# 0xPolygonZero/plonky

Measured on AMD Instinct MI355X. Metric: MSM Mpairs/sec + NTT Melems/sec, 2^20 Tweedledee, 1/2/4/8 GPU, higher is better.
Workload: dtype u32; 1 GPU; 2^20 TweedledeeBase forward NTT + 2^20-pair tweedledee MSM per GPU per step; log_n=20, curve=tweedledee

## Files before the change

### plonky_amd/csrc/msm_order.hip

```cpp
#include "msm_dev.cuh"
#include "glv.cuh"
#include <cstdlib>

namespace plk {


struct OrdRaw {
    uint4 lo, hi;
};
PLK_DI OrdRaw ord_load_scalar(const uint4* __restrict__ scalars, size_t i, bool live) {
    OrdRaw r;
    r.lo = r.hi = make_uint4(0u, 0u, 0u, 0u);
    if (live) {
        r.lo = scalars[i * 2];
        r.hi = scalars[i * 2 + 1];
    }
    return r;
}
template <class SP> PLK_DI void ord_park_loaded(const OrdRaw& r, uint32_t* s_lim, int tid, bool raw_signed) {
    static_assert(SP::NL == 8, "scalar fields are 256-bit");
    Fe<SP> s;
    s.v[0] = r.lo.x; s.v[1] = r.lo.y; s.v[2] = r.lo.z; s.v[3] = r.lo.w;
    s.v[4] = r.hi.x; s.v[5] = r.hi.y; s.v[6] = r.hi.z; s.v[7] = r.hi.w;
    if (!raw_signed) s = fe_to_canonical<SP>(s);
// ... 486 lines not shown
    __syncthreads();
    const uint32_t last_total = s_bins[nbins - 1];
    block_excl_scan4(s_bins, nbins, s_sum);
    for (int k = threadIdx.x; k < nbins; k += 256) bin_base[k] = s_bins[k];
    if (threadIdx.x == 0) {
        const uint32_t total = s_bins[nbins - 1] + last_total;
        bin_base[nbins] = total;
        uint32_t ch = lanes_cfg ? (total + lanes_cfg - 1) / lanes_cfg : chunk_cfg;
        if (ch < 8u) ch = 8u;
        if (ch > chunk_cfg) ch = chunk_cfg;
        dyn_chunk[0] = ch;
    }
    __syncthreads();
    for (int k = threadIdx.x; k < nbins; k += 256) s_bins[k] = s_tot[k] > hot ? (s_tot[k] + ORD_SEG - 1) / ORD_SEG : 0u;
    __syncthreads();
    const uint32_t last_segs = s_bins[nbins - 1];
    block_excl_scan4(s_bins, nbins, s_sum);
    for (int k = threadIdx.x; k < nbins; k += 256) seg_base[k] = s_bins[k];
    if (threadIdx.x == 0) seg_base[nbins] = s_bins[nbins - 1] + last_segs;
}

struct Ord2Seg {
    uint32_t bin, seg, plo, phi;
};
PLK_DI bool ord2_segment(const uint32_t* __restrict__ seg_base, const uint32_t* __restrict__ bin_base, int nbins, uint32_t blk, Ord2Seg& sg) {
    if (blk >= seg_base[nbins]) return false;
    uint32_t a = 0, b = (uint32_t)nbins;
    while (b - a > 1) {
        const uint32_t m = (a + b) >> 1;
        if (seg_base[m] <= blk) a = m; else b = m;
    }
    sg.bin = a;
    sg.seg = blk - seg_base[a];
    sg.plo = sg.seg * ORD_SEG;
    sg.phi = min(bin_base[a + 1] - bin_base[a], sg.plo + ORD_SEG);
    return true;
}
PLK_DI void ord2_prefix(const uint32_t* __restrict__ cnt1, uint32_t nt, uint32_t bin, uint32_t* s_run, uint32_t* s_pre, uint32_t* s_tmp) {
    const int tid = threadIdx.x, nthr = blockDim.x;
    const uint32_t per = (nt + nthr - 1) / nthr;
    const uint32_t lo = min(nt, (uint32_t)tid * per), hi = min(nt, lo + per);
    uint32_t sum = 0;
    for (uint32_t t = lo; t < hi; ++t) {
        const uint32_t w = cnt1[(size_t)bin * nt + t];
        s_run[t] = w;
        sum += w & 0xFFFFu;
    }
    uint32_t total = 0;
    uint32_t run = block_excl_prefix(sum, s_tmp, &total);
    for (uint32_t t = lo; t < hi; ++t) {
        s_pre[t] = run;
        run += s_run[t] & 0xFFFFu;
    }
    if (tid == 0) {
        s_pre[nt] = total;
        s_run[nt] = 0;
    }
    __syncthreads();
}
template <int THREADS = ORD_BIN_THREADS, int EPT = ORD_SEG_EPT>
PLK_DI void ord2_gather(const uint32_t* __restrict__ tmp, const uint32_t* s_run, const uint32_t* s_pre, uint32_t nt, uint32_t cap, uint32_t plo, uint32_t phi,
                        uint32_t (&rec)[EPT], uint32_t (&til)[EPT]) {
    uint32_t t[EPT];
#pragma unroll
    for (int k = 0; k < EPT; ++k) t[k] = 0;
    uint32_t top = 1;
    while (top * 2 <= nt) top *= 2;
    for (uint32_t step = top; step; step >>= 1) {
#pragma unroll
        for (int k = 0; k < EPT; ++k) {
            const uint32_t p = plo + threadIdx.x + (uint32_t)k * THREADS;
            const uint32_t cand = t[k] + step;
            if (cand < nt && s_pre[cand] <= p) t[k] = cand;
        }
    }
#pragma unroll
    for (int k = 0; k < EPT; ++k) {
        const uint32_t p = plo + threadIdx.x + (uint32_t)k * THREADS;
        til[k] = t[k];
        rec[k] = 0;
        if (p < phi) rec[k] = tmp[(size_t)t[k] * cap + (s_run[t[k]] >> 16) + (p - s_pre[t[k]])];
    }
}
__global__ void __launch_bounds__(ORD_BIN_THREADS) k_ord_bin_count2(const uint32_t* __restrict__ tmp, const uint32_t* __restrict__ cnt1, uint32_t nt, uint32_t cap,
                                                                    const uint32_t* __restrict__ bin_base, const uint32_t* __restrict__ seg_base, int fine_bits,
                                                                    int nbins, uint32_t* __restrict__ cnt2) {
    __shared__ uint32_t s_hist[1 << ORD_MAX_FINE];
    __shared__ uint32_t s_tmp[ORD_BIN_THREADS];
    extern __shared__ __attribute__((aligned(16))) uint32_t s_dyn[];
    uint32_t* s_run = s_dyn;
    uint32_t* s_pre = s_dyn + (nt + 1);
    const int tid = threadIdx.x;
    const int nf = 1 << fine_bits;
    const uint32_t fmask = (uint32_t)nf - 1u;
    for (uint32_t blk = blockIdx.x;; blk += gridDim.x) {
        Ord2Seg sg;
        if (!ord2_segment(seg_base, bin_base, nbins, blk, sg)) return;
        for (int k = tid; k < nf; k += ORD_BIN_THREADS) s_hist[k] = 0;
        ord2_prefix(cnt1, nt, sg.bin, s_run, s_pre, s_tmp);
        uint32_t rec[ORD_SEG_EPT], til[ORD_SEG_EPT];
        ord2_gather(tmp, s_run, s_pre, nt, cap, sg.plo, sg.phi, rec, til);
#pragma unroll
        for (int k = 0; k < ORD_SEG_EPT; ++k)
            if (sg.plo + tid + k * ORD_BIN_THREADS < sg.phi) atomicAdd(&s_hist[(rec[k] >> 1) & fmask], 1u);
        __syncthreads();
        for (int k = tid; k < nf; k += ORD_BIN_THREADS) cnt2[((size_t)blk << fine_bits) + k] = s_hist[k];
        __syncthreads();
    }
}
__global__ void __launch_bounds__(ORD_BIN_THREADS) k_ord_bin_scatter2(const uint32_t* __restrict__ tmp, const uint32_t* __restrict__ cnt1, uint32_t nt, uint32_t cap,
                                                                      const uint32_t* __restrict__ bin_base, const uint32_t* __restrict__ seg_base, int fine_bits,
                                                                      int nbins, uint32_t buckets, const uint32_t* __restrict__ cnt2, uint32_t* __restrict__ off,
                                                                      uint32_t* __restrict__ sorted, uint32_t entries_cap, uint32_t ent_stride, uint32_t ent_first) {
    __shared__ uint32_t s_tmp[ORD_BIN_THREADS];
    __shared__ uint32_t s_out[ORD_SEG];
    __shared__ uint16_t s_fine[ORD_SEG];
    extern __shared__ __attribute__((aligned(16))) uint32_t s_dyn[];
    uint32_t* s_glob = s_dyn;
    uint32_t* s_loc = s_dyn + ((size_t)1 << fine_bits);
    uint32_t* s_cur = s_dyn + ((size_t)2 << fine_bits);
    uint32_t* s_run = s_dyn + ((size_t)3 << fine_bits);
    uint32_t* s_pre = s_run + (nt + 1);
    const int tid = threadIdx.x;
    for (uint32_t blk = blockIdx.x;; blk += gridDim.x) {
    Ord2Seg sg;
    if (!ord2_segment(seg_base, bin_base, nbins, blk, sg)) return;
    const int nf = 1 << fine_bits;
    const uint32_t fmask = (uint32_t)nf - 1u;
    const uint32_t bin = sg.bin, seg = sg.seg;
    ord2_prefix(cnt1, nt, bin, s_run, s_pre, s_tmp);
    uint32_t rec[ORD_SEG_EPT], til[ORD_SEG_EPT];
    ord2_gather(tmp, s_run, s_pre, nt, cap, sg.plo, sg.phi, rec, til);
    const uint32_t s0 = seg_base[bin], s1 = seg_base[bin + 1];
    for (int k = tid; k < nf; k += ORD_BIN_THREADS) {
        uint32_t tot = 0, before = 0, own = 0;
        for (uint32_t sgi = s0; sgi < s1; ++sgi) {
            const uint32_t v = cnt2[((size_t)sgi << fine_bits) + k];
            if (sgi - s0 < seg) before += v;
            if (sgi - s0 == seg) own = v;
            tot += v;
        }
        s_glob[k] = tot;
        s_cur[k] = before;
        s_loc[k] = own;
    }
    __syncthreads();
    block_excl_scan4(s_glob, nf, s_tmp);
    block_excl_scan4(s_loc, nf, s_tmp);
    const uint32_t bb = bin_base[bin];
    for (int k = tid; k < nf; k += ORD_BIN_THREADS) {
        const uint32_t o = bb + s_glob[k];
        if (seg == 0) off[((size_t)bin << fine_bits) + k] = o;
        s_glob[k] = o + s_cur[k];
        s_cur[k] = s_loc[k];
    }
    __syncthreads();
#pragma unroll
    for (int k = 0; k < ORD_SEG_EPT; ++k) {
        if (sg.plo + tid + k * ORD_BIN_THREADS >= sg.phi) continue;
        const uint32_t r = rec[k];
        const uint32_t f = (r >> 1) & fmask;
        const uint32_t idx = atomicAdd(&s_cur[f], 1u);
        if (PLK_CHK(idx < ORD_SEG, CHK_SEG_STAGE)) {
            const uint32_t entry = ((r >> 12) & 15u) * ent_stride + ent_first + til[k] * (uint32_t)ORD2_TS + (r >> 16);
            s_out[idx] = (entry << 1) | (r & 1u);
            s_fine[idx] = (uint16_t)f;
        }
    }
    __syncthreads();
    const uint32_t count = sg.phi - sg.plo;
    for (uint32_t i = tid; i < count; i += ORD_BIN_THREADS) {
        const uint32_t f = s_fine[i];
        const uint32_t at = s_glob[f] + (i - s_loc[f]);
        if (PLK_CHK(at < entries_cap, CHK_SORTED_INDEX)) sorted[at] = s_out[i];
    }
    __syncthreads();
    }
}

constexpr int ORD2_SORT_THREADS = 1024;
constexpr int ORD2_SORT_UNROLL = 8;
template <class F>
PLK_DI void ord2_for_runs(const uint32_t* __restrict__ tmp, const uint32_t* s_run, uint32_t nt, uint32_t cap, F&& f) {
    const uint32_t hw = threadIdx.x >> 5, hl = threadIdx.x & 31u;
    constexpr uint32_t HW = ORD2_SORT_THREADS / 32;
    for (uint32_t t0 = hw; t0 < nt; t0 += HW * ORD2_SORT_UNROLL) {
        uint32_t w[ORD2_SORT_UNROLL], r[ORD2_SORT_UNROLL];
#pragma unroll
        for (int u = 0; u < ORD2_SORT_UNROLL; ++u) {
            const uint32_t t = t0 + (uint32_t)u * HW;
            w[u] = t < nt ? s_run[t] : 0u;
            r[u] = 0;
            if (hl < (w[u] & 0xFFFFu)) r[u] = tmp[(size_t)t * cap + (w[u] >> 16) + hl];
        }
#pragma unroll
        for (int u = 0; u < ORD2_SORT_UNROLL; ++u) {
            const uint32_t t = t0 + (uint32_t)u * HW, cnt = w[u] & 0xFFFFu;
            if (hl < cnt) f(r[u], t);
            for (uint32_t i = hl + 32u; i < cnt; i += 32u) f(tmp[(size_t)t * cap + (w[u] >> 16) + i], t);
        }
    }
}
template <bool CACHE>
__global__ void __launch_bounds__(ORD2_SORT_THREADS) k_ord_bin_sort(const uint32_t* __restrict__ tmp, const uint32_t* __restrict__ cnt1, uint32_t nt, uint32_t cap,
                                                                    const uint32_t* __restrict__ bin_base, int fine_bits, int nbins, uint32_t buckets,
                                                                    uint32_t* __restrict__ off, uint32_t* __restrict__ sorted, uint32_t entries_cap,
                                                                    uint32_t ent_stride, uint32_t ent_first) {
    __shared__ uint32_t s_tmp[ORD2_SORT_THREADS];
    extern __shared__ __attribute__((aligned(16))) uint32_t s_dyn[];
    const int nf = 1 << fine_bits;
    uint32_t* s_out = s_dyn;
    uint32_t* s_cur = s_dyn + ORD2_BIN_CAP;
    uint32_t* s_run = s_cur + nf;
    const int tid = threadIdx.x;
    const uint32_t bin = blockIdx.x;
    const uint32_t bb = bin_base[bin], total = bin_base[bin + 1] - bb;
    if (bin == 0 && tid == 0) off[buckets] = bin_base[nbins];
    if (total == 0) {
        for (int k = tid; k < nf; k += ORD2_SORT_THREADS) off[((size_t)bin << fine_bits) + k] = bb;
        return;
    }
    if (total > ORD2_BIN_CAP) return;
    const uint32_t fmask = (uint32_t)nf - 1u;
    for (int k = tid; k < nf; k += ORD2_SORT_THREADS) s_cur[k] = 0;
    for (uint32_t t = tid; t < nt; t += ORD2_SORT_THREADS) s_run[t] = cnt1[(size_t)bin * nt + t];
    __syncthreads();
    auto count = [&](uint32_t r, uint32_t) { atomicAdd(&s_cur[(r >> 1) & fmask], 1u); };
    auto place = [&](uint32_t r, uint32_t t) {
        const uint32_t idx = atomicAdd(&s_cur[(r >> 1) & fmask], 1u);
        const uint32_t entry = ((r >> 12) & 15u) * ent_stride + ent_first + t * (uint32_t)ORD2_TS + (r >> 16);
        if (PLK_CHK(idx < ORD2_BIN_CAP, CHK_SEG_STAGE)) s_out[idx] = (entry << 1) | (r & 1u);
    };
    constexpr int STEPS = 4;
    constexpr uint32_t HW = ORD2_SORT_THREADS / 32;
    const uint32_t hw = (uint32_t)tid >> 5, hl = (uint32_t)tid & 31u;
    uint32_t rc[STEPS * ORD2_SORT_UNROLL];
    if constexpr (CACHE) {
#pragma unroll
        for (int st = 0; st < STEPS; ++st) {
#pragma unroll
            for (int u = 0; u < ORD2_SORT_UNROLL; ++u) {
                const uint32_t t = hw + (uint32_t)(st * ORD2_SORT_UNROLL + u) * HW;
                const uint32_t w = t < nt ? s_run[t] : 0u;
                rc[st * ORD2_SORT_UNROLL + u] = 0;
                if (hl < (w & 0xFFFFu)) rc[st * ORD2_SORT_UNROLL + u] = tmp[(size_t)t * cap + (w >> 16) + hl];
            }
#pragma unroll
            for (int u = 0; u < ORD2_SORT_UNROLL; ++u) {
                const uint32_t t = hw + (uint32_t)(st * ORD2_SORT_UNROLL + u) * HW;
                const uint32_t w = t < nt ? s_run[t] : 0u, cnt = w & 0xFFFFu;
                if (hl < cnt) count(rc[st * ORD2_SORT_UNROLL + u], t);
                for (uint32_t i = hl + 32u; i < cnt; i += 32u) count(tmp[(size_t)t * cap + (w >> 16) + i], t);
            }
        }
    } else {
        ord2_for_runs(tmp, s_run, nt, cap, count);
    }
    __syncthreads();
    block_excl_scan4(s_cur, nf, s_tmp);
    for (int k = tid; k < nf; k += ORD2_SORT_THREADS) off[((size_t)bin << fine_bits) + k] = bb + s_cur[k];
    __syncthreads();
    if constexpr (CACHE) {
#pragma unroll
        for (int st = 0; st < STEPS; ++st)
#pragma unroll
            for (int u = 0; u < ORD2_SORT_UNROLL; ++u) {
                const uint32_t t = hw + (uint32_t)(st * ORD2_SORT_UNROLL + u) * HW;
                const uint32_t w = t < nt ? s_run[t] : 0u, cnt = w & 0xFFFFu;
                if (hl < cnt) place(rc[st * ORD2_SORT_UNROLL + u], t);
                for (uint32_t i = hl + 32u; i < cnt; i += 32u) place(tmp[(size_t)t * cap + (w >> 16) + i], t);
            }
    } else {
        ord2_for_runs(tmp, s_run, nt, cap, place);
    }
    __syncthreads();
    for (uint32_t i = tid; i < total; i += ORD2_SORT_THREADS)
        if (PLK_CHK(bb + i < entries_cap, CHK_SORTED_INDEX)) sorted[bb + i] = s_out[i];
}

template <class C> int msm_launch_glv_split(const void* d_scalars, size_t n, void* halves, hipStream_t stream) {
    k_glv_split<C><<<(unsigned)((n + 255) / 256), 256, 0, stream>>>((const uint4*)d_scalars, n, (uint4*)halves);
    PLK_HIP_TRY(hipGetLastError());
    return PLK_OK;
}
static bool order_tiles2(const OrdCfg& o) { return o.perm != 0; }
template <class C> int msm_launch_order_stage(int stage, const OrdCfg& o, const OrdBuffers& b, hipStream_t stream) {
    const bool one_level = o.fine_bits == 0;
    if (order_tiles2(o)) {
        const uint32_t cap = (uint32_t)ORD2_TS * (uint32_t)o.windows;
        if (stage == 0) {
            const size_t lds = (size_t)cap * 4;
            (void)hipFuncSetAttribute((const void*)k_ord_tiles<C>, hipFuncAttributeMaxDynamicSharedMemorySize, ORD2_TS * ORD2_MAX_WINDOWS * 4);
            k_ord_tiles<C><<<o.nt1, ORD2_THREADS, lds, stream>>>((const uint4*)b.scalars, b.n, o, (uint32_t*)b.cnt1, b.bin_total, (uint32_t*)b.tmp);
            k_ord_scan_bins<<<1, 256, 0, stream>>>(b.bin_total, o.nbins, b.bin_base, b.seg_base, b.done_counter + 2, b.chunk, b.lanes, ORD2_BIN_CAP);
        } else if (stage == 2) {
            const size_t entries = b.n * (size_t)o.windows;
            const size_t hot_bins = entries / ORD2_BIN_CAP < (size_t)o.nbins ? entries / ORD2_BIN_CAP : (size_t)o.nbins;
            const unsigned segs = (unsigned)(entries / ORD_SEG + hot_bins + 1);
            const size_t lds = (size_t)2 * (o.nt1 + 1) * 4, lds_s = lds + ((size_t)3 << o.fine_bits) * 4;
            const size_t lds_b = ((size_t)ORD2_BIN_CAP + ((size_t)1 << o.fine_bits) + o.nt1) * 4;
            static const bool no_cache = getenv("PLK_MSM_BINSORT_NOCACHE") != nullptr;
            if (o.nt1 <= 1024u && !no_cache) {
                (void)hipFuncSetAttribute((const void*)k_ord_bin_sort<true>, hipFuncAttributeMaxDynamicSharedMemorySize, (int)lds_b);
                k_ord_bin_sort<true><<<o.nbins, ORD2_SORT_THREADS, lds_b, stream>>>((const uint32_t*)b.tmp, (const uint32_t*)b.cnt1, o.nt1, cap, b.bin_base, o.fine_bits,
                                                                                   o.nbins, b.buckets, (uint32_t*)b.off, (uint32_t*)b.sorted, o.entries_cap, o.ent_stride,
                                                                                   o.ent_first);
            } else {
                (void)hipFuncSetAttribute((const void*)k_ord_bin_sort<false>, hipFuncAttributeMaxDynamicSharedMemorySize, (int)lds_b);
                k_ord_bin_sort<false><<<o.nbins, ORD2_SORT_THREADS, lds_b, stream>>>((const uint32_t*)b.tmp, (const uint32_t*)b.cnt1, o.nt1, cap, b.bin_base, o.fine_bits,
                                                                                    o.nbins, b.buckets, (uint32_t*)b.off, (uint32_t*)b.sorted, o.entries_cap, o.ent_stride,
                                                                                    o.ent_first);
            }
            const unsigned hot_grid = segs < 512u ? segs : 512u;
            k_ord_bin_count2<<<hot_grid, ORD_BIN_THREADS, lds, stream>>>((const uint32_t*)b.tmp, (const uint32_t*)b.cnt1, o.nt1, cap, b.bin_base, b.seg_base, o.fine_bits,
                                                                   o.nbins, (uint32_t*)b.cnt2);
            k_ord_bin_scatter2<<<hot_grid, ORD_BIN_THREADS, lds_s, stream>>>((const uint32_t*)b.tmp, (const uint32_t*)b.cnt1, o.nt1, cap, b.bin_base, b.seg_base,
                                                                               o.fine_bits, o.nbins, b.buckets, (const uint32_t*)b.cnt2, (uint32_t*)b.off,
                                                                               (uint32_t*)b.sorted, o.entries_cap, o.ent_stride, o.ent_first);
        }
        PLK_HIP_TRY(hipGetLastError());
        return PLK_OK;
    }
    if (stage == 0) {
        k_ord_count<C><<<o.nt1, ORD_THREADS, 0, stream>>>((const uint4*)b.scalars, b.n, o, (uint32_t*)b.cnt1);
        k_ord_scan1<<<o.nbins, 256, 0, stream>>>((uint32_t*)b.cnt1, o.nt1, o.nbins, b.bin_total, b.bin_base, b.seg_base, b.done_counter, b.done_counter + 2,
                                                 b.chunk, b.lanes, one_level ? (uint32_t*)b.off : nullptr);
    } else if (stage == 1) {
        k_ord_scatter<C><<<o.nt1, ORD_THREADS, 0, stream>>>((const uint4*)b.scalars, b.n, o, (const uint32_t*)b.cnt1, b.bin_base, (uint2*)b.tmp,
                                                            one_level ? (uint32_t*)b.sorted : nullptr);
    } else if (!one_level) {
        const unsigned segs = (unsigned)(b.n * (size_t)o.windows / ORD_SEG + o.nbins + 1);
        k_ord_bin_count<<<segs, ORD_BIN_THREADS, 0, stream>>>((const uint2*)b.tmp, b.bin_base, b.seg_base, o.fine_bits, o.nbins, (uint32_t*)b.cnt2);
        k_ord_bin_scatter<<<segs + o.nbins, ORD_BIN_THREADS, 0, stream>>>((const uint2*)b.tmp, b.bin_base, b.seg_base, o.fine_bits, o.nbins, b.buckets,
                                                                          (const uint32_t*)b.cnt2, (uint32_t*)b.off, (uint32_t*)b.sorted, o.entries_cap);
    }
    PLK_HIP_TRY(hipGetLastError());
    return PLK_OK;
}
template <class C> int msm_launch_digits(const void* d_scalars, size_t n, const OrdCfg& o, void* d_digits, hipStream_t stream) {
    k_ord_digits<C><<<(unsigned)((n + ORD_THREADS - 1) / ORD_THREADS), ORD_THREADS, 0, stream>>>((const uint4*)d_scalars, n, o, (int32_t*)d_digits);
    PLK_HIP_TRY(hipGetLastError());
    return PLK_OK;
}
#define PLK_ORD_INSTANTIATE(C)                                                                     \
    template int msm_launch_glv_split<C>(const void*, size_t, void*, hipStream_t);                \
    template int msm_launch_order_stage<C>(int, const OrdCfg&, const OrdBuffers&, hipStream_t);   \
    template int msm_launch_digits<C>(const void*, size_t, const OrdCfg&, void*, hipStream_t);
PLK_ORD_INSTANTIATE(TweedledeeCurve)
PLK_ORD_INSTANTIATE(TweedledumCurve)
PLK_ORD_INSTANTIATE(Bls12377Curve)
PLK_ORD_INSTANTIATE(PallasCurve)
PLK_ORD_INSTANTIATE(VestaCurve)
#undef PLK_ORD_INSTANTIATE

PLK_CHK_READER(msm_order_checked_failures)

}
```

### plonky_amd/csrc/msm_tail.hip

```cpp
#include "msm_dev.cuh"
#include "ecz_coop.cuh"
#include <cstdlib>

namespace plk {

template <class FP> PLK_DI void emit_result(const XyzzZ<FP>& acc, const TailSlot& sl) {
    if (sl.projective) emit_projective<FP>(acc, sl.out_xy, sl.out_zero);
    else emit_affine<FP, true>(acc, sl.out_xy, sl.out_zero);
}

template <class FP> PLK_DI XyzzZ<FP> wave_sum(XyzzZ<FP> v, int width) {
    for (int m = 1; m < width; m <<= 1) v = xyzzz_add<FP>(v, xyzzz_shfl_xor<FP>(v, m));
    return v;
}


PLK_DI bool bucket_heads(const uint32_t* __restrict__ off, uint32_t b, uint32_t chunk, uint32_t& first, uint32_t& count) {
    const uint32_t o0 = off[b], o1 = off[b + 1];
    first = 0;
    count = 0;
    if (o1 == o0) return false;
    const uint32_t l0 = o0 / chunk, l1 = (o1 - 1) / chunk;
    first = l0 + 1;
    count = l1 - l0;
    return true;
}

__global__ void __launch_bounds__(256) k_msm_heavy_list(TailBatch tb, uint32_t buckets, uint32_t cap, int lpb_log) {
    const uint32_t* __restrict__ off = tb.s[blockIdx.y].off;
    const uint32_t chunk = tb.s[blockIdx.y].dyn_chunk[0];
    uint32_t* __restrict__ heavy = tb.s[blockIdx.y].heavy;
    const uint32_t b = blockIdx.x * blockDim.x + threadIdx.x;
    if (b >= buckets) return;
    uint32_t first, ns;
    bucket_heads(off, b, chunk, first, ns);
    if (ns <= (HEAVY_HEADS << lpb_log)) return;
    const uint32_t chunks = (ns + HEAVY_CHUNK - 1) / HEAVY_CHUNK;
    const uint32_t at = atomicAdd(&heavy[0], chunks);
    const uint32_t hb = atomicAdd(&heavy[1], 1u);
    if (hb < cap) heavy[2 + 2 * cap + hb] = b;
    for (uint32_t k = 0; k < chunks; ++k)
        if (at + k < cap) {
            heavy[2 + 2 * (at + k)] = b;
            heavy[3 + 2 * (at + k)] = k;
        }
}

template <class FP> PLK_DI XyzzZ<FP> block256_sum(XyzzZ<FP> acc, uint4* s_pts) {
    constexpr int RU = raw_u4<FP>();
    acc = wave_sum<FP>(acc, 64);
    const int wave = threadIdx.x >> 6, lane = threadIdx.x & 63;
    if (lane == 0) xyzzz_store_raw<FP>(s_pts + wave * RU, acc);
    __syncthreads();
    acc = (wave == 0 && lane < 4) ? xyzzz_load_raw<FP>(s_pts + lane * RU) : xyzzz_identity<FP>();
    if (wave == 0) acc = wave_sum<FP>(acc, 4);
    __syncthreads();
    return acc;
}

template <class C>
__global__ void __launch_bounds__(256) k_msm_heavy_chunks(TailBatch tb, uint32_t cap) {
    using FP = typename C::FP;
    constexpr int RU = raw_u4<FP>();
    __shared__ uint4 s_pts[4 * RU];
    const uint32_t chunk = tb.s[blockIdx.y].dyn_chunk[0];
    const uint4* __restrict__ p_head = tb.s[blockIdx.y].p_head;
    const uint32_t* __restrict__ off = tb.s[blockIdx.y].off;
    const uint32_t* __restrict__ heavy = tb.s[blockIdx.y].heavy;
    uint4* __restrict__ heavy_part = tb.s[blockIdx.y].heavy_part;
    const uint32_t items = min(heavy[0], cap);
    for (uint32_t it = blockIdx.x; it < items; it += gridDim.x) {
        const uint32_t b = heavy[2 + 2 * it], k = heavy[3 + 2 * it];
        uint32_t first, ns;
        bucket_heads(off, b, chunk, first, ns);
        const uint32_t s0 = first + k * HEAVY_CHUNK, s1 = min(first + ns, s0 + HEAVY_CHUNK);
        XyzzZ<FP> acc = xyzzz_identity<FP>();
        for (uint32_t s = s0 + threadIdx.x; s < s1; s += 256)
            if (tb.s[blockIdx.y].head_live[s]) acc = xyzzz_add<FP>(acc, xyzzz_load_raw<FP>(p_head + (size_t)s * RU));
        acc = block256_sum<FP>(acc, s_pts);
        if (threadIdx.x == 0) xyzzz_store_raw<FP>(heavy_part + (size_t)it * RU, acc);
    }
}
template <class C>
__global__ void __launch_bounds__(256) k_msm_heavy_final(TailBatch tb, uint32_t cap) {
    using FP = typename C::FP;
    constexpr int RU = raw_u4<FP>();
    __shared__ uint4 s_pts[4 * RU];
    const uint32_t* __restrict__ heavy = tb.s[blockIdx.y].heavy;
    const uint4* __restrict__ heavy_part = tb.s[blockIdx.y].heavy_part;
    uint4* __restrict__ p_start = tb.s[blockIdx.y].p_start;
    const uint32_t items = min(heavy[0], cap), nb = min(heavy[1], cap);
    for (uint32_t hb = blockIdx.x; hb < nb; hb += gridDim.x) {
        const uint32_t b = heavy[2 + 2 * cap + hb];
        XyzzZ<FP> acc = threadIdx.x == 0 ? xyzzz_load_raw<FP>(p_start + (size_t)b * RU) : xyzzz_identity<FP>();
        for (uint32_t it = threadIdx.x; it < items; it += 256)
            if (heavy[2 + 2 * it] == b) acc = xyzzz_add<FP>(acc, xyzzz_load_raw<FP>(heavy_part + (size_t)it * RU));
        acc = block256_sum<FP>(acc, s_pts);
        if (threadIdx.x == 0) xyzzz_store_raw<FP>(p_start + (size_t)b * RU, acc);
    }
}

template <class C, bool PACKED>
__global__ void __launch_bounds__(256) k_msm_assemble(TailBatch tb, uint32_t buckets, int lpb_log) {
    using FP = typename C::FP;
    constexpr int W = FP::NL / 4;
    constexpr int RU = raw_u4<FP>();
    const TailSlot& sl = tb.s[blockIdx.y];
    const uint32_t chunk = sl.dyn_chunk[0];
    if (blockIdx.x == 0 && threadIdx.x < 2) sl.heavy[threadIdx.x] = 0;
    if (blockIdx.x == 0 && threadIdx.x == 2) *sl.final_done = 0;
    if (blockIdx.x == 0 && threadIdx.x == 3) *sl.live_count = 0;
    const uint32_t gid = blockIdx.x * blockDim.x + threadIdx.x;
    const uint32_t b = gid >> lpb_log, part = gid & ((1u << lpb_log) - 1u);
    XyzzZ<FP> acc = xyzzz_identity<FP>();
    bool nonempty = false, touched = false;
    if (b < buckets) {
        uint32_t first, ns;
        nonempty = bucket_heads(sl.off, b, chunk, first, ns);
        uint32_t live = 0;
        if (ns <= (HEAVY_HEADS << lpb_log))
            for (uint32_t h = part; h < ns; h += 1u << lpb_log) live |= sl.head_live[first + h] ? (1u << (h >> lpb_log)) : 0u;
        touched = live != 0;
        if (lpb_log > 0 || PACKED || touched) {
            if (nonempty && part == 0) acc = xyzzz_load_raw<FP>(sl.p_start + (size_t)b * RU);
            for (uint32_t h = part, k = 0; h < ns && live; h += 1u << lpb_log, ++k)
                if ((live >> k) & 1u) acc = xyzzz_add<FP>(acc, xyzzz_load_raw<FP>(sl.p_head + (size_t)(first + h) * RU));
        }
    }
    if (lpb_log > 0) acc = wave_sum<FP>(acc, 1 << lpb_log);
    if (b < buckets && part == 0) {
        if constexpr (PACKED) xyzzz_store_packed<FP>(sl.bucket + (size_t)b * 4 * W, acc);
        else if (lpb_log > 0 || touched || !nonempty) xyzzz_store_raw<FP>(sl.p_start + (size_t)b * RU, acc);
    }
}

template <class C>
__global__ void __launch_bounds__(256) k_msm_heads(TailBatch tb, uint32_t buckets, uint32_t cap) {
    using FP = typename C::FP;
    constexpr int RU = raw_u4<FP>();
    const TailSlot& sl = tb.s[blockIdx.y];
    if (blockIdx.x == 0 && threadIdx.x == 0) *sl.final_done = 0;
    const int ql = threadIdx.x & 3;
    const uint32_t quads = gridDim.x * (blockDim.x >> 2);
    const uint32_t nlive = *sl.live_count;
    const uint32_t chunk = sl.dyn_chunk[0];
    for (uint32_t item = blockIdx.x * (blockDim.x >> 2) + (threadIdx.x >> 2); item < nlive; item += quads) {
        const uint32_t l = sl.live_list[item];
        const uint32_t b = sl.head_bucket[l];
        if (b >= buckets) continue;
        uint32_t first, ns;
        bucket_heads(sl.off, b, chunk, first, ns);
        if (l < first || l >= first + ns) continue;
        if (ns > HEAVY_HEADS) {
            if (l == first && ql == 0) {
                uint32_t* __restrict__ heavy = sl.heavy;
                const uint32_t chunks = (ns + HEAVY_CHUNK - 1) / HEAVY_CHUNK;
                const uint32_t at = atomicAdd(&heavy[0], chunks);
                const uint32_t hb = atomicAdd(&heavy[1], 1u);
                if (hb < cap) heavy[2 + 2 * cap + hb] = b;
                for (uint32_t k = 0; k < chunks; ++k)
                    if (at + k < cap) {
                        heavy[2 + 2 * (at + k)] = b;
                        heavy[3 + 2 * (at + k)] = k;
                    }
            }
            continue;
        }
        bool leader = true;
        for (uint32_t h = first; h < l; ++h) leader = leader && !sl.head_live[h];
        if (!leader) continue;
        XyzzZ<FP> acc = xyzzz_load_raw<FP>(sl.p_start + (size_t)b * RU);
        for (uint32_t h = l; h < first + ns; ++h)
            if (h == l || sl.head_live[h]) acc = xyzzz_add_q<FP>(acc, xyzzz_load_raw<FP>(sl.p_head + (size_t)h * RU), ql);
        if (ql == 0) xyzzz_store_raw<FP>(sl.p_start + (size_t)b * RU, acc);
    }
}

template <class C>
__global__ void __launch_bounds__(128) k_msm_gsum(TailBatch tb, int L, int H, int g_log, int reset_heavy) {
    using FP = typename C::FP;
    constexpr int RU = raw_u4<FP>();
    const TailSlot& sl = tb.s[blockIdx.y];
    const uint32_t nbg = (1u << (L + H)) >> g_log;
    const uint32_t t = blockIdx.x * blockDim.x + threadIdx.x;
    if (reset_heavy && blockIdx.x == 0 && blockIdx.z == 0 && threadIdx.x < 2) sl.heavy[threadIdx.x] = 0;
    if (reset_heavy && blockIdx.x == 0 && blockIdx.z == 0 && threadIdx.x == 2) *sl.live_count = 0;
    if (t >= 2 * nbg) return;
    const uint32_t wbase = blockIdx.z << (L + H);
    uint4* part = sl.line_part + (size_t)blockIdx.z * 2 * nbg * RU;
    const uint32_t G = 1u << g_log;
    uint32_t b0, bstep;
    uint4* dst;
    if (t < nbg) {
        const uint32_t pr = (1u << L) >> g_log;
        const uint32_t hi = t / pr, g = t % pr;
        b0 = wbase + (hi << L) + (g << g_log);
        bstep = 1;
        dst = part + (size_t)t * RU;
    } else {
        const uint32_t u = t - nbg;
        const uint32_t lo = u & ((1u << L) - 1u), g = u >> L;
        const uint32_t pc = (1u << H) >> g_log;
        b0 = wbase + ((g << g_log) << L) + lo;
        bstep = 1u << L;
        dst = part + ((size_t)nbg + (size_t)lo * pc + g) * RU;
    }
    const uint32_t* __restrict__ off = sl.off;
    auto load_bucket = [&](uint32_t b) {
        if (off[b + 1] == off[b]) return xyzzz_identity<FP>();
        return xyzzz_load_raw<FP>(sl.p_start + (size_t)b * RU);
    };
    XyzzZ<FP> acc = xyzzz_identity<FP>();
    XyzzZ<FP> nxt = load_bucket(b0);
    for (uint32_t k = 0; k < G; ++k) {
        XyzzZ<FP> cur = nxt;
        const uint32_t b = b0 + k * bstep;
        if (k + 1 < G) nxt = load_bucket(b + bstep);
        acc = xyzzz_add<FP>(acc, cur);
    }
    xyzzz_store_raw<FP>(dst, acc);
}

template <class C, int LV>
__global__ void __launch_bounds__(128) k_msm_gsum_tree(TailBatch tb, int L, int H, int g_log) {
    using FP = typename C::FP;
    constexpr int RU = raw_u4<FP>();
    __shared__ uint4 s_a[128 * RU], s_b[64 * RU];
    const TailSlot& sl = tb.s[blockIdx.y];
    const int tid = threadIdx.x;
    if (blockIdx.x == 0 && blockIdx.z == 0 && tid < 2) sl.heavy[tid] = 0;
    if (blockIdx.x == 0 && blockIdx.z == 0 && tid == 2) *sl.live_count = 0;
    const uint32_t nbg = (1u << (L + H)) >> g_log;
    const uint32_t row_blocks = nbg >> 7;
    const uint32_t wbase = blockIdx.z << (L + H);
    uint4* part = sl.line_part + (size_t)blockIdx.z * 2 * (nbg >> LV) * RU;
    const uint32_t G = 1u << g_log;
    const bool rows = blockIdx.x < row_blocks;
    uint32_t b0, bstep;
    if (rows) {
        const uint32_t t = blockIdx.x * 128u + tid;
        const uint32_t pr = (1u << L) >> g_log;
        b0 = wbase + ((t / pr) << L) + ((t % pr) << g_log);
        bstep = 1;
    } else {
        const uint32_t cb = blockIdx.x - row_blocks, sets = (1u << L) >> 4;
        const uint32_t lo = ((cb % sets) << 4) + (tid & 15), g = ((cb / sets) << 3) + (tid >> 4);
        b0 = wbase + ((g << g_log) << L) + lo;
        bstep = 1u << L;
// ... 160 lines not shown
                }
            }
        }
    }
}

template <class C>
__global__ void __launch_bounds__(FINAL_THREADS) k_msm_final_pair(TailBatch tb, int parts, int planes, int pair_shift) {
    using FP = typename C::FP;
    constexpr int W = FP::NL / 4;
    constexpr int RU = raw_u4<FP>();
    static_assert(FINAL_THREADS == 512, "two windows of 256 threads");
    __shared__ uint4 s_pts[2 * 33 * 4 * W];
    __shared__ uint4 s_x[RU];
    const int tid = threadIdx.x, ql = tid & 3, half = (tid >> 6) & 1, ltid = ((tid >> 7) << 6) | (tid & 63), item = ltid >> 2;
    const int slot = blockIdx.x;
    const uint4* __restrict__ plane_part = tb.s[slot].plane_part;
    const int ipq = parts > 1 ? 2 : 1, qpp = parts / ipq;
    const int plane = item / qpp, sub = item % qpp;
    const bool live = plane < planes;
    const uint4* src = plane_part + ((size_t)(half * planes + plane) * parts + sub * ipq) * 4 * W;
    uint4* sp = s_pts + half * 33 * 4 * W;
    XyzzZ<FP> acc = live ? xyzzz_load_packed<FP>(src) : xyzzz_identity<FP>();
    if (ipq == 2) acc = xyzzz_add_q<FP>(acc, live ? xyzzz_load_packed<FP>(src + 4 * W) : xyzzz_identity<FP>(), ql);
    acc = wave_sum_q<FP>(acc, qpp, ql);
    if (live && sub == 0) {
        for (int k = 0; k < plane; ++k) acc = xyzzz_dbl_q<FP>(acc, ql);
        if (ql == 0) xyzzz_store_packed<FP>(sp + plane * 4 * W, acc);
    }
    __syncthreads();
    if (ltid < 128) {
        acc = item < planes ? xyzzz_load_packed<FP>(sp + item * 4 * W) : xyzzz_identity<FP>();
        acc = wave_sum_q<FP>(acc, 16, ql);
        if (ltid == 64) xyzzz_store_packed<FP>(sp + 32 * 4 * W, acc);
    }
    __syncthreads();
    if (ltid < 4) {
        if (planes > 16) acc = xyzzz_add_q<FP>(acc, xyzzz_load_packed<FP>(sp + 32 * 4 * W), ql);
        if (half == 1) {
            for (int k = 0; k < pair_shift; ++k) acc = xyzzz_dbl_q<FP>(acc, ql);
            if (ql == 0) xyzzz_store_raw<FP>(s_x, acc);
        }
    }
    __syncthreads();
    if (tid < 4) {
        acc = xyzzz_add_q<FP>(acc, xyzzz_load_raw<FP>(s_x), ql);
        if (tid == 0) emit_result<FP>(acc, tb.s[slot]);
    }
}

template <class C>
__global__ void __launch_bounds__(COMBINE_THREADS) k_msm_combine(TailBatch tb, int windows) {
    using FP = typename C::FP;
    constexpr int W = FP::NL / 4;
    __shared__ uint4 s_pts[(COMBINE_THREADS / 64) * 4 * W];
    const uint4* __restrict__ win_pts = tb.s[blockIdx.x].win_pts;
    const int tid = threadIdx.x, ql = tid & 3, item = tid >> 2;
    XyzzZ<FP> acc = item < windows ? xyzzz_load_packed<FP>(win_pts + (size_t)item * 4 * W) : xyzzz_identity<FP>();
    acc = wave_sum_q<FP>(acc, 16, ql);
    if ((tid & 63) == 0) xyzzz_store_packed<FP>(s_pts + (tid >> 6) * 4 * W, acc);
    __syncthreads();
    if (tid < 64) {
        acc = item < COMBINE_THREADS / 64 ? xyzzz_load_packed<FP>(s_pts + item * 4 * W) : xyzzz_identity<FP>();
        acc = wave_sum_q<FP>(acc, COMBINE_THREADS / 64, ql);
        if (tid == 0) emit_result<FP>(acc, tb.s[blockIdx.x]);
    }
}

#ifdef PLK_FINAL_TRACE
extern "C" int plk_debug_final_trace(unsigned long long* out) {
    return hipMemcpyFromSymbol(out, HIP_SYMBOL(g_final_trace), sizeof(unsigned long long) * 32) == hipSuccess ? 0 : -1;
}
#endif

template <class C> int msm_launch_reduce_stage(int stage, const TailGeom& g, const TailBatch& tb, hipStream_t stream) {
    const uint32_t buckets = g.buckets;
    const unsigned cnt = (unsigned)tb.count;
    const int tw = g.tail_windows;
    static const bool tail_v1 = getenv("PLK_MSM_TAIL_V1") != nullptr;
    const bool v2 = g.two_level && g.lpb_log == 0 && !tail_v1;
    if (stage == 0) {
        if (v2) k_msm_heads<C><<<dim3(g.many_heads ? 2048 : 512, cnt), 256, 0, stream>>>(tb, buckets, g.heavy_cap);
        else k_msm_heavy_list<<<dim3((buckets + 255) / 256, cnt), 256, 0, stream>>>(tb, buckets, g.heavy_cap, g.lpb_log);
        k_msm_heavy_chunks<C><<<dim3(256, cnt), 256, 0, stream>>>(tb, g.heavy_cap);
        k_msm_heavy_final<C><<<dim3(64, cnt), 256, 0, stream>>>(tb, g.heavy_cap);
        const unsigned ab = (unsigned)((((size_t)buckets << g.lpb_log) + 255) / 256);
        const int Lm = g.transposed ? g.H : g.L, Hm = g.transposed ? g.L : g.H;
        if (v2) {
            const uint32_t nbg = (1u << (g.L + g.H)) >> g.g_log;
            const unsigned wins = g.table_free ? (unsigned)g.windows : 1u;
            static const int tree_env = getenv("PLK_MSM_TREE") ? atoi(getenv("PLK_MSM_TREE")) : 2;
            int lv = tree_env;
            if (g.L - g.g_log < 3 || g.H - g.g_log < 3 || Lm < 4 || nbg < 128) lv = 0;
            if (lv >= 3) k_msm_gsum_tree<C, 3><<<dim3(2 * (nbg >> 7), cnt, wins), 128, 0, stream>>>(tb, Lm, Hm, g.g_log);
            else if (lv == 2) k_msm_gsum_tree<C, 2><<<dim3(2 * (nbg >> 7), cnt, wins), 128, 0, stream>>>(tb, Lm, Hm, g.g_log);
            else k_msm_gsum<C><<<dim3((2 * nbg + 127) / 128, cnt, wins), 128, 0, stream>>>(tb, Lm, Hm, g.g_log, 1);
            const int g2 = g.g_log + (lv >= 3 ? 3 : lv == 2 ? 2 : 0);
            const int longest = (g.H > g.L ? g.H : g.L) - g2, qpl = longest < 4 ? longest : 4;
            const size_t lanes2 = ((size_t)2 << g.H) << (qpl + 2);
            k_msm_lsum<C><<<dim3((unsigned)((lanes2 + 255) / 256), cnt, wins), 256, 0, stream>>>(tb, g.L, g.H, g2, qpl, g.transposed);
        } else if (g.two_level) {
            const uint32_t nbg = (1u << (g.L + g.H)) >> g.g_log;
            const unsigned wins = g.table_free ? (unsigned)g.windows : 1u;
            k_msm_assemble<C, false><<<dim3(ab, cnt), 256, 0, stream>>>(tb, buckets, g.lpb_log);
            k_msm_gsum<C><<<dim3((2 * nbg + 127) / 128, cnt, wins), 128, 0, stream>>>(tb, Lm, Hm, g.g_log, 0);
            const size_t lanes = ((size_t)2 << g.H) << (g.lpl_log + 2);
            k_msm_lsum<C><<<dim3((unsigned)((lanes + 255) / 256), cnt, wins), 256, 0, stream>>>(tb, g.L, g.H, g.g_log, g.lpl_log, g.transposed);
        } else {
            k_msm_assemble<C, true><<<dim3(ab, cnt), 256, 0, stream>>>(tb, buckets, g.lpb_log);
        }
    } else if (stage == 1) {
        dim3 pg(g.plane_blocks, g.planes, tw * cnt);
        k_msm_planes<C><<<pg, PLANE_THREADS, 0, stream>>>(tb, tw, g.tail_wbuckets);
    } else {
        static const bool final_v1 = getenv("PLK_MSM_FINAL_V1") != nullptr || tail_v1;
        const int qpp = g.plane_blocks > 1 ? g.plane_blocks / 2 : 1;
        if (g.two_level && !g.table_free && tw == 2 && g.planes * qpp <= 64 && g.planes <= 32 && !final_v1) {
            k_msm_final_pair<C><<<cnt, FINAL_THREADS, 0, stream>>>(tb, g.plane_blocks, g.planes, g.L);
        } else {
            k_msm_final<C><<<tw * cnt, FINAL_THREADS, 0, stream>>>(tb, tw, g.plane_blocks, g.planes, g.tail_shift, g.two_level ? g.L : -1);
            if (tw > FINAL_FUSE_WINDOWS) k_msm_combine<C><<<cnt, COMBINE_THREADS, 0, stream>>>(tb, tw);
        }
    }
    PLK_HIP_TRY(hipGetLastError());
    return PLK_OK;
}
template int msm_launch_reduce_stage<TweedledeeCurve>(int, const TailGeom&, const TailBatch&, hipStream_t);
template int msm_launch_reduce_stage<TweedledumCurve>(int, const TailGeom&, const TailBatch&, hipStream_t);
template int msm_launch_reduce_stage<Bls12377Curve>(int, const TailGeom&, const TailBatch&, hipStream_t);
template int msm_launch_reduce_stage<PallasCurve>(int, const TailGeom&, const TailBatch&, hipStream_t);
template int msm_launch_reduce_stage<VestaCurve>(int, const TailGeom&, const TailBatch&, hipStream_t);

}
```

Baseline: 1508 M units/s (1 unit = 1 NTT element or 1 MSM scalar-point pair; components below).

## Fuse bin-count into bin-sort launch and merge heavy-bucket chunk/final kernels

The hot-segment count kernel now runs as extra blocks prepended to the bin-sort grid, so one launch does both jobs and the count overlaps the per-bin sorts. In the MSM tail, the heavy-chunk and heavy-final kernels become one kernel. Single-chunk buckets add straight into p_start, and for multi-chunk buckets the last-arriving chunk, found by an atomic counter with threadfences, does the final reduction. This removes two kernel launches and their serialization, at the cost of a larger LDS allocation for the fused sort kernel and an extra counter slot per heavy-list entry.

After: 1522 M units/s (1 unit = 1 NTT element or 1 MSM scalar-point pair; components below), median of 6. No clear change (+1.0%).

```diff
diff --git a/plonky_amd/csrc/msm_order.hip b/plonky_amd/csrc/msm_order.hip
--- a/plonky_amd/csrc/msm_order.hip
+++ b/plonky_amd/csrc/msm_order.hip
@@ -592,29 +592,29 @@
         if (p < phi) rec[k] = tmp[(size_t)t[k] * cap + (s_run[t[k]] >> 16) + (p - s_pre[t[k]])];
     }
 }
-__global__ void __launch_bounds__(ORD_BIN_THREADS) k_ord_bin_count2(const uint32_t* __restrict__ tmp, const uint32_t* __restrict__ cnt1, uint32_t nt, uint32_t cap,
-                                                                    const uint32_t* __restrict__ bin_base, const uint32_t* __restrict__ seg_base, int fine_bits,
-                                                                    int nbins, uint32_t* __restrict__ cnt2) {
-    __shared__ uint32_t s_hist[1 << ORD_MAX_FINE];
-    __shared__ uint32_t s_tmp[ORD_BIN_THREADS];
-    extern __shared__ __attribute__((aligned(16))) uint32_t s_dyn[];
-    uint32_t* s_run = s_dyn;
-    uint32_t* s_pre = s_dyn + (nt + 1);
+template <int THREADS>
+PLK_DI void ord2_count_segments(const uint32_t* __restrict__ tmp, const uint32_t* __restrict__ cnt1, uint32_t nt, uint32_t cap,
+                                const uint32_t* __restrict__ bin_base, const uint32_t* __restrict__ seg_base, int fine_bits, int nbins,
+                                uint32_t* __restrict__ cnt2, uint32_t first_blk, uint32_t grid, uint32_t* s_dyn, uint32_t* s_tmp) {
+    constexpr int EPT = (int)(ORD_SEG / THREADS);
     const int tid = threadIdx.x;
     const int nf = 1 << fine_bits;
     const uint32_t fmask = (uint32_t)nf - 1u;
-    for (uint32_t blk = blockIdx.x;; blk += gridDim.x) {
+    uint32_t* s_hist = s_dyn;
+    uint32_t* s_run = s_dyn + nf;
+    uint32_t* s_pre = s_run + (nt + 1);
+    for (uint32_t blk = first_blk;; blk += grid) {
         Ord2Seg sg;
         if (!ord2_segment(seg_base, bin_base, nbins, blk, sg)) return;
-        for (int k = tid; k < nf; k += ORD_BIN_THREADS) s_hist[k] = 0;
+        for (int k = tid; k < nf; k += THREADS) s_hist[k] = 0;
         ord2_prefix(cnt1, nt, sg.bin, s_run, s_pre, s_tmp);
-        uint32_t rec[ORD_SEG_EPT], til[ORD_SEG_EPT];
-        ord2_gather(tmp, s_run, s_pre, nt, cap, sg.plo, sg.phi, rec, til);
-#pragma unroll
-        for (int k = 0; k < ORD_SEG_EPT; ++k)
-            if (sg.plo + tid + k * ORD_BIN_THREADS < sg.phi) atomicAdd(&s_hist[(rec[k] >> 1) & fmask], 1u);
-        __syncthreads();
-        for (int k = tid; k < nf; k += ORD_BIN_THREADS) cnt2[((size_t)blk << fine_bits) + k] = s_hist[k];
+        uint32_t rec[EPT], til[EPT];
+        ord2_gather<THREADS, EPT>(tmp, s_run, s_pre, nt, cap, sg.plo, sg.phi, rec, til);
+#pragma unroll
+        for (int k = 0; k < EPT; ++k)
+            if (sg.plo + tid + k * THREADS < sg.phi) atomicAdd(&s_hist[(rec[k] >> 1) & fmask], 1u);
+        __syncthreads();
+        for (int k = tid; k < nf; k += THREADS) cnt2[((size_t)blk << fine_bits) + k] = s_hist[k];
         __syncthreads();
     }
 }
@@ -713,7 +713,8 @@
 }
 template <bool CACHE>
 __global__ void __launch_bounds__(ORD2_SORT_THREADS) k_ord_bin_sort(const uint32_t* __restrict__ tmp, const uint32_t* __restrict__ cnt1, uint32_t nt, uint32_t cap,
-                                                                    const uint32_t* __restrict__ bin_base, int fine_bits, int nbins, uint32_t buckets,
+                                                                    const uint32_t* __restrict__ bin_base, const uint32_t* __restrict__ seg_base,
+                                                                    int fine_bits, int nbins, uint32_t buckets, uint32_t count_grid, uint32_t* __restrict__ cnt2,
                                                                     uint32_t* __restrict__ off, uint32_t* __restrict__ sorted, uint32_t entries_cap,
                                                                     uint32_t ent_stride, uint32_t ent_first) {
     __shared__ uint32_t s_tmp[ORD2_SORT_THREADS];
@@ -723,7 +724,11 @@
     uint32_t* s_cur = s_dyn + ORD2_BIN_CAP;
     uint32_t* s_run = s_cur + nf;
     const int tid = threadIdx.x;
-    const uint32_t bin = blockIdx.x;
+    if (blockIdx.x < count_grid) {
+        ord2_count_segments<ORD2_SORT_THREADS>(tmp, cnt1, nt, cap, bin_base, seg_base, fine_bits, nbins, cnt2, blockIdx.x, count_grid, s_dyn, s_tmp);
+        return;
+    }
+    const uint32_t bin = blockIdx.x - count_grid;
     const uint32_t bb = bin_base[bin], total = bin_base[bin + 1] - bb;
     if (bin == 0 && tid == 0) off[buckets] = bin_base[nbins];
     if (total == 0) {
@@ -808,22 +813,22 @@
             const size_t hot_bins = entries / ORD2_BIN_CAP < (size_t)o.nbins ? entries / ORD2_BIN_CAP : (size_t)o.nbins;
             const unsigned segs = (unsigned)(entries / ORD_SEG + hot_bins + 1);
             const size_t lds = (size_t)2 * (o.nt1 + 1) * 4, lds_s = lds + ((size_t)3 << o.fine_bits) * 4;
-            const size_t lds_b = ((size_t)ORD2_BIN_CAP + ((size_t)1 << o.fine_bits) + o.nt1) * 4;
+            const unsigned hot_grid = segs < 512u ? segs : 512u;
+            const unsigned count_grid = segs < 256u ? segs : 256u;
+            size_t lds_b = ((size_t)ORD2_BIN_CAP + ((size_t)1 << o.fine_bits) + o.nt1) * 4;
+            if (lds_b < lds + ((size_t)4 << o.fine_bits)) lds_b = lds + ((size_t)4 << o.fine_bits);
             static const bool no_cache = getenv("PLK_MSM_BINSORT_NOCACHE") != nullptr;
             if (o.nt1 <= 1024u && !no_cache) {
                 (void)hipFuncSetAttribute((const void*)k_ord_bin_sort<true>, hipFuncAttributeMaxDynamicSharedMemorySize, (int)lds_b);
-                k_ord_bin_sort<true><<<o.nbins, ORD2_SORT_THREADS, lds_b, stream>>>((const uint32_t*)b.tmp, (const uint32_t*)b.cnt1, o.nt1, cap, b.bin_base, o.fine_bits,
-                                                                                   o.nbins, b.buckets, (uint32_t*)b.off, (uint32_t*)b.sorted, o.entries_cap, o.ent_stride,
-                                                                                   o.ent_first);
+                k_ord_bin_sort<true><<<count_grid + (unsigned)o.nbins, ORD2_SORT_THREADS, lds_b, stream>>>(
+                    (const uint32_t*)b.tmp, (const uint32_t*)b.cnt1, o.nt1, cap, b.bin_base, b.seg_base, o.fine_bits, o.nbins, b.buckets, count_grid,
+                    (uint32_t*)b.cnt2, (uint32_t*)b.off, (uint32_t*)b.sorted, o.entries_cap, o.ent_stride, o.ent_first);
             } else {
                 (void)hipFuncSetAttribute((const void*)k_ord_bin_sort<false>, hipFuncAttributeMaxDynamicSharedMemorySize, (int)lds_b);
-                k_ord_bin_sort<false><<<o.nbins, ORD2_SORT_THREADS, lds_b, stream>>>((const uint32_t*)b.tmp, (const uint32_t*)b.cnt1, o.nt1, cap, b.bin_base, o.fine_bits,
-                                                                                    o.nbins, b.buckets, (uint32_t*)b.off, (uint32_t*)b.sorted, o.entries_cap, o.ent_stride,
-                                                                                    o.ent_first);
+                k_ord_bin_sort<false><<<count_grid + (unsigned)o.nbins, ORD2_SORT_THREADS, lds_b, stream>>>(
+                    (const uint32_t*)b.tmp, (const uint32_t*)b.cnt1, o.nt1, cap, b.bin_base, b.seg_base, o.fine_bits, o.nbins, b.buckets, count_grid,
+                    (uint32_t*)b.cnt2, (uint32_t*)b.off, (uint32_t*)b.sorted, o.entries_cap, o.ent_stride, o.ent_first);
             }
-            const unsigned hot_grid = segs < 512u ? segs : 512u;
-            k_ord_bin_count2<<<hot_grid, ORD_BIN_THREADS, lds, stream>>>((const uint32_t*)b.tmp, (const uint32_t*)b.cnt1, o.nt1, cap, b.bin_base, b.seg_base, o.fine_bits,
-                                                                   o.nbins, (uint32_t*)b.cnt2);
             k_ord_bin_scatter2<<<hot_grid, ORD_BIN_THREADS, lds_s, stream>>>((const uint32_t*)b.tmp, (const uint32_t*)b.cnt1, o.nt1, cap, b.bin_base, b.seg_base,
                                                                                o.fine_bits, o.nbins, b.buckets, (const uint32_t*)b.cnt2, (uint32_t*)b.off,
                                                                                (uint32_t*)b.sorted, o.entries_cap, o.ent_stride, o.ent_first);
diff --git a/plonky_amd/csrc/msm_tail.hip b/plonky_amd/csrc/msm_tail.hip
--- a/plonky_amd/csrc/msm_tail.hip
+++ b/plonky_amd/csrc/msm_tail.hip
@@ -26,6 +26,16 @@
     return true;
 }
 
+PLK_DI void heavy_list_bucket(uint32_t* __restrict__ heavy, uint32_t b, uint32_t ns, uint32_t cap) {
+    const uint32_t chunks = (ns + HEAVY_CHUNK - 1) / HEAVY_CHUNK;
+    const uint32_t at = atomicAdd(&heavy[0], chunks);
+    for (uint32_t k = 0; k < chunks; ++k)
+        if (at + k < cap) {
+            heavy[2 + 3 * (at + k)] = b;
+            heavy[3 + 3 * (at + k)] = k;
+            heavy[4 + 3 * (at + k)] = 0;
+        }
+}
 __global__ void __launch_bounds__(256) k_msm_heavy_list(TailBatch tb, uint32_t buckets, uint32_t cap, int lpb_log) {
     const uint32_t* __restrict__ off = tb.s[blockIdx.y].off;
     const uint32_t chunk = tb.s[blockIdx.y].dyn_chunk[0];
@@ -35,15 +45,7 @@
     uint32_t first, ns;
     bucket_heads(off, b, chunk, first, ns);
     if (ns <= (HEAVY_HEADS << lpb_log)) return;
-    const uint32_t chunks = (ns + HEAVY_CHUNK - 1) / HEAVY_CHUNK;
-    const uint32_t at = atomicAdd(&heavy[0], chunks);
-    const uint32_t hb = atomicAdd(&heavy[1], 1u);
-    if (hb < cap) heavy[2 + 2 * cap + hb] = b;
-    for (uint32_t k = 0; k < chunks; ++k)
-        if (at + k < cap) {
-            heavy[2 + 2 * (at + k)] = b;
-            heavy[3 + 2 * (at + k)] = k;
-        }
+    heavy_list_bucket(heavy, b, ns, cap);
 }
 
 template <class FP> PLK_DI XyzzZ<FP> block256_sum(XyzzZ<FP> acc, uint4* s_pts) {
@@ -59,18 +61,20 @@
 }
 
 template <class C>
-__global__ void __launch_bounds__(256) k_msm_heavy_chunks(TailBatch tb, uint32_t cap) {
+__global__ void __launch_bounds__(256) k_msm_heavy(TailBatch tb, uint32_t cap) {
     using FP = typename C::FP;
     constexpr int RU = raw_u4<FP>();
     __shared__ uint4 s_pts[4 * RU];
+    __shared__ uint32_t s_last;
     const uint32_t chunk = tb.s[blockIdx.y].dyn_chunk[0];
     const uint4* __restrict__ p_head = tb.s[blockIdx.y].p_head;
     const uint32_t* __restrict__ off = tb.s[blockIdx.y].off;
-    const uint32_t* __restrict__ heavy = tb.s[blockIdx.y].heavy;
+    uint32_t* __restrict__ heavy = tb.s[blockIdx.y].heavy;
     uint4* __restrict__ heavy_part = tb.s[blockIdx.y].heavy_part;
+    uint4* __restrict__ p_start = tb.s[blockIdx.y].p_start;
     const uint32_t items = min(heavy[0], cap);
     for (uint32_t it = blockIdx.x; it < items; it += gridDim.x) {
-        const uint32_t b = heavy[2 + 2 * it], k = heavy[3 + 2 * it];
+        const uint32_t b = heavy[2 + 3 * it], k = heavy[3 + 3 * it];
         uint32_t first, ns;
         bucket_heads(off, b, chunk, first, ns);
         const uint32_t s0 = first + k * HEAVY_CHUNK, s1 = min(first + ns, s0 + HEAVY_CHUNK);
@@ -78,25 +82,24 @@
         for (uint32_t s = s0 + threadIdx.x; s < s1; s += 256)
             if (tb.s[blockIdx.y].head_live[s]) acc = xyzzz_add<FP>(acc, xyzzz_load_raw<FP>(p_head + (size_t)s * RU));
         acc = block256_sum<FP>(acc, s_pts);
-        if (threadIdx.x == 0) xyzzz_store_raw<FP>(heavy_part + (size_t)it * RU, acc);
-    }
-}
-template <class C>
-__global__ void __launch_bounds__(256) k_msm_heavy_final(TailBatch tb, uint32_t cap) {
-    using FP = typename C::FP;
-    constexpr int RU = raw_u4<FP>();
-    __shared__ uint4 s_pts[4 * RU];
-    const uint32_t* __restrict__ heavy = tb.s[blockIdx.y].heavy;
-    const uint4* __restrict__ heavy_part = tb.s[blockIdx.y].heavy_part;
-    uint4* __restrict__ p_start = tb.s[blockIdx.y].p_start;
-    const uint32_t items = min(heavy[0], cap), nb = min(heavy[1], cap);
-    for (uint32_t hb = blockIdx.x; hb < nb; hb += gridDim.x) {
-        const uint32_t b = heavy[2 + 2 * cap + hb];
-        XyzzZ<FP> acc = threadIdx.x == 0 ? xyzzz_load_raw<FP>(p_start + (size_t)b * RU) : xyzzz_identity<FP>();
-        for (uint32_t it = threadIdx.x; it < items; it += 256)
-            if (heavy[2 + 2 * it] == b) acc = xyzzz_add<FP>(acc, xyzzz_load_raw<FP>(heavy_part + (size_t)it * RU));
-        acc = block256_sum<FP>(acc, s_pts);
-        if (threadIdx.x == 0) xyzzz_store_raw<FP>(p_start + (size_t)b * RU, acc);
+        const uint32_t at = it - k, chunks = min((ns + HEAVY_CHUNK - 1) / HEAVY_CHUNK, cap - at);
+        if (chunks == 1) {
+            if (threadIdx.x == 0) xyzzz_store_raw<FP>(p_start + (size_t)b * RU, xyzzz_add<FP>(xyzzz_load_raw<FP>(p_start + (size_t)b * RU), acc));
+            continue;
+        }
+        if (threadIdx.x == 0) {
+            xyzzz_store_raw<FP>(heavy_part + (size_t)it * RU, acc);
+            __threadfence();
+            s_last = atomicAdd(&heavy[4 + 3 * at], 1u) == chunks - 1u;
+        }
+        __syncthreads();
+        if (s_last) {
+            __threadfence();
+            acc = threadIdx.x == 0 ? xyzzz_load_raw<FP>(p_start + (size_t)b * RU) : xyzzz_identity<FP>();
+            for (uint32_t j = threadIdx.x; j < chunks; j += 256) acc = xyzzz_add<FP>(acc, xyzzz_load_raw<FP>(heavy_part + (size_t)(at + j) * RU));
+            acc = block256_sum<FP>(acc, s_pts);
+            if (threadIdx.x == 0) xyzzz_store_raw<FP>(p_start + (size_t)b * RU, acc);
+        }
     }
 }
 
@@ -152,18 +155,7 @@
         bucket_heads(sl.off, b, chunk, first, ns);
         if (l < first || l >= first + ns) continue;
         if (ns > HEAVY_HEADS) {
-            if (l == first && ql == 0) {
-                uint32_t* __restrict__ heavy = sl.heavy;
-                const uint32_t chunks = (ns + HEAVY_CHUNK - 1) / HEAVY_CHUNK;
-                const uint32_t at = atomicAdd(&heavy[0], chunks);
-                const uint32_t hb = atomicAdd(&heavy[1], 1u);
-                if (hb < cap) heavy[2 + 2 * cap + hb] = b;
-                for (uint32_t k = 0; k < chunks; ++k)
-                    if (at + k < cap) {
-                        heavy[2 + 2 * (at + k)] = b;
-                        heavy[3 + 2 * (at + k)] = k;
-                    }
-            }
+            if (l == first && ql == 0) heavy_list_bucket(sl.heavy, b, ns, cap);
             continue;
         }
         bool leader = true;
@@ -490,8 +482,7 @@
     if (stage == 0) {
         if (v2) k_msm_heads<C><<<dim3(g.many_heads ? 2048 : 512, cnt), 256, 0, stream>>>(tb, buckets, g.heavy_cap);
         else k_msm_heavy_list<<<dim3((buckets + 255) / 256, cnt), 256, 0, stream>>>(tb, buckets, g.heavy_cap, g.lpb_log);
-        k_msm_heavy_chunks<C><<<dim3(256, cnt), 256, 0, stream>>>(tb, g.heavy_cap);
-        k_msm_heavy_final<C><<<dim3(64, cnt), 256, 0, stream>>>(tb, g.heavy_cap);
+        k_msm_heavy<C><<<dim3(256, cnt), 256, 0, stream>>>(tb, g.heavy_cap);
         const unsigned ab = (unsigned)((((size_t)buckets << g.lpb_log) + 255) / 256);
         const int Lm = g.transposed ? g.H : g.L, Hm = g.transposed ? g.L : g.H;
         if (v2) {
```
